# s-will/BiAlign

Measured on AMD Instinct MI355X. Metric: giga-DP-cells/sec, higher is better.
Workload: dtype int32

## Files before the change

bialign_amd/csrc/bialign_host.hpp:

```cpp
#pragma once
#include "bialign_plan.hpp"

#include <algorithm>
#include <cstdarg>
#include <cstdio>
#include <cstdlib>
#include <cstring>
#include <memory>
#include <mutex>
#include <numeric>
#include <string>
#include <type_traits>
#include <vector>

namespace bialign {

#define HIP_TRY(expr)                                                                 \
  do {                                                                                \
    hipError_t e_ = (expr);                                                           \
    if (e_ != hipSuccess)                                                             \
      return fail(BIALIGN_E_DEVICE, "%s failed: %s (%s:%d)", #expr, hipGetErrorString(e_), \
                  __FILE__, __LINE__);                                                \
  } while (0)

template <typename T>
struct DevBuf {
  T* p = nullptr;
  size_t n = 0;
  ~DevBuf() { release(); }
  void release() {
    if (p) (void)hipFree(p);
    p = nullptr;
    n = 0;
  }
  void swap(DevBuf& o) {
    std::swap(p, o.p);
    std::swap(n, o.n);
  }
  hipError_t alloc(size_t count) {
    release();
    n = count;
    return hipMalloc(reinterpret_cast<void**>(&p), std::max<size_t>(count, 1) * sizeof(T));
  }
  hipError_t upload(const T* src, size_t count, hipStream_t s) {
    hipError_t e = alloc(count);
    if (e != hipSuccess || count == 0) return e;
    return hipMemcpyAsync(p, src, count * sizeof(T), hipMemcpyHostToDevice, s);
  }
};

}

using bialign::DevBuf;
using bialign::DeviceBatch;
using bialign::PairDesc;
using bialign::TraceState;

struct bialign_engine {
  int device = 0;
  int num_cu = 256;
  hipStream_t stream = nullptr;
  hipStream_t copy_stream = nullptr;
  hipEvent_t ev[4] = {nullptr, nullptr, nullptr, nullptr};
  int live_batches = 0;
  bool closing = false;
  DevBuf<int32_t> layer_cache;
  DevBuf<int32_t> layer_cache2;
  DevBuf<int32_t> tab_cache;
};

struct bialign_batch : bialign::BatchPlan {
  bialign_engine* eng = nullptr;
  DevBuf<PairDesc> d_pairs;
  DevBuf<int32_t> d_order, d_s1, d_s2, d_layers, d_scores, d_tlen, d_complete, d_err, d_prog;
  DevBuf<int32_t> d_span;
  DevBuf<unsigned long long> d_end_key;
  int last_team = 1;
  int xcu_resident[4] = {-1, -1, -1, -1};
  bool used_xcu = false;
  bool no_xcu = false;
  int recovered = 0;
  int xcu_spin_limit = 1 << 20;
  uint32_t pending_flags = 0;
  bool used_pack = false;
  bool packed_layers = false;
  DevBuf<uint8_t> d_seq_a, d_cls_a, d_seq_b, d_cls_b, d_trace;
  DevBuf<int32_t> d_tab;
  DevBuf<double> d_feat_a, d_feat_b;
  int64_t feat_tot_a = 0, feat_tot_b = 0;
  DevBuf<int32_t> d_mu1;
  DevBuf<int64_t> d_mu1_off;
  std::vector<hipEvent_t> build_evs;
  double build_ms = 0;
  int build_launches = 0;
  DevBuf<uint8_t> d_null_seq, d_null_cls;
  DevBuf<int64_t> d_null_off;
  DevBuf<double> d_null_feat;
  DevBuf<int32_t> d_null_tab;
  DevBuf<int64_t> d_null_tab_off;
  DevBuf<uint16_t> d_null_perm;
  DevBuf<int32_t> d_null_obs;
  DevBuf<bialign_null_stats> d_null_stats;
  hipEvent_t null_evs[4] = {nullptr, nullptr, nullptr, nullptr};
  double shuffle_ms = 0, stats_ms = 0;
  int32_t null_model = BIALIGN_NULL_MONO;
  DevBuf<TraceState> d_tstate;
  bool hits_on = false;
  bialign_hit_spec hit_spec{};
  DevBuf<int32_t> d_hit_profile, d_hit_head, d_hit_rec, d_hit_walks;
  DevBuf<int64_t> d_hit_prof_off;
  DevBuf<uint8_t> d_hit_trace;
  std::vector<int64_t> hit_prof_off;
  int hit_mask_words = 0;
  int64_t hit_bytes = 0;
  std::vector<hipEvent_t> hit_evs;
  bool hits_pending = false;
  bool hits_ran = false;
  double search_ms = 0;
  void release_hits() {
    hits_on = hits_ran = false;
    for (DevBuf<int32_t>* d : {&d_hit_profile, &d_hit_head, &d_hit_rec, &d_hit_walks}) d->release();
    d_hit_prof_off.release();
    d_hit_trace.release();
    hit_bytes = 0;
  }
  bialign_timing timing{};
  bool ran = false, ran_trace = false;
  bool pending = false, pending_trace = false;
  std::vector<hipEvent_t> evs;
  hipEvent_t uploaded = nullptr;
  ~bialign_batch() {
    for (hipEvent_t e : evs)
      if (e) (void)hipEventDestroy(e);
    for (hipEvent_t e : build_evs)
      if (e) (void)hipEventDestroy(e);
    for (hipEvent_t e : null_evs)
      if (e) (void)hipEventDestroy(e);
    for (hipEvent_t e : hit_evs)
      if (e) (void)hipEventDestroy(e);
    if (uploaded) (void)hipEventDestroy(uploaded);
  }

  DeviceBatch view() const {
    DeviceBatch v{};
    v.pairs = d_pairs.p;
    v.order = d_order.p;
    v.seq_a = d_seq_a.p; v.cls_a = d_cls_a.p; v.seq_b = d_seq_b.p; v.cls_b = d_cls_b.p;
    v.s1 = d_s1.p; v.s2 = d_s2.p;
    v.k1 = k1; v.k2 = k2;
    v.beta = prm.gap_opening_cost; v.gamma = prm.gap_cost; v.delta = prm.shift_cost;
    v.layers = d_layers.p;
    v.scores = d_scores.p;
    v.trace = d_trace.p;
    v.trace_len = d_tlen.p;
    v.complete = d_complete.p;
    v.errflag = d_err.p;
    v.dense_tab = (dense || dense1) ? d_tab.p : nullptr;
    v.dense_forms = (dense ? 1 : 0) | (dense1 ? 2 : 0);
    v.scratch = d_layers.p;
    v.wide_ring = ring_dwords.empty() ? nullptr : d_layers.p + max_chunk_dwords;
    v.wide_score_only = !ring_dwords.empty() && lean ? 1 : 0;
    v.tstate = d_tstate.p;
    v.resw_k = level_trace ? wide_seg : resw_k;
    v.wide_s = S;
    v.prio_mode = getenv("BIALIGN_PRIO") ? atoi(getenv("BIALIGN_PRIO")) : 1;
    v.spin_limit = 1 << 20;
    v.free_ends = mode == bialign::AlignMode::Fit       ? bialign::FREE_B_ENDS
                  : mode == bialign::AlignMode::Overlap ? bialign::FREE_B_ENDS | bialign::FREE_A_ENDS
                                                        : 0;
    v.local = mode == bialign::AlignMode::Local;
    v.reserved0 = nullptr;
    v.span = d_span.p;
    v.end_key = d_end_key.p;
    return v;
  }
};

namespace bialign {

int xcu_serial_begin(bialign_engine* e);
int xcu_serial_end(bialign_engine* e);

int launch_build_mu2(bialign_batch* b, int first, int count);

int launch_shuffle_null(bialign_batch* b, int first, int count);
int launch_permute_tables(bialign_batch* b, int first, int count);
int launch_null_stats(bialign_batch* b, const int32_t* d_observed);

template <typename... P>
hipError_t allow_lds(void (*kern)(P...), size_t lds) {
  if (lds <= 64 * 1024) return hipSuccess;
  return hipFuncSetAttribute(reinterpret_cast<const void*>(kern), hipFuncAttributeMaxDynamicSharedMemorySize, (int)lds);
}
template <typename... P, typename... A>
hipError_t try_launch(void (*kern)(P...), dim3 grid, dim3 block, size_t lds, hipStream_t st, const A&... args) {
  if (hipError_t e = allow_lds(kern, lds)) return e;
  hipLaunchKernelGGL(kern, grid, block, lds, st, args...);
  return hipGetLastError();
}
template <typename... P, typename... A>
int launch(void (*kern)(P...), dim3 grid, dim3 block, size_t lds, hipStream_t st, const A&... args) {
  HIP_TRY(try_launch(kern, grid, block, lds, st, args...));
  return BIALIGN_OK;
}

template <typename... P, typename... X>
int launch_team(bialign_batch* b, void (*kern)(P...), dim3 grid, dim3 block, size_t lds, DeviceBatch w, int count,
                bool serial, const X&... extra) {
  const size_t words = (size_t)count * PROG_WORDS;
  if (b->d_prog.n < words) HIP_TRY(b->d_prog.alloc(words));
  HIP_TRY(hipMemsetAsync(b->d_prog.p, 0, words * sizeof(int32_t), b->eng->stream));
  w.prog = b->d_prog.p;
  w.spin_limit = b->xcu_spin_limit;
  if (!serial) return launch(kern, grid, block, lds, b->eng->stream, w, extra...);
  b->used_xcu = true;
  if (int rc = xcu_serial_begin(b->eng)) return rc;
  const hipError_t launched = try_launch(kern, grid, block, lds, b->eng->stream, w, extra...);
  const int rc = xcu_serial_end(b->eng);
  if (launched == hipSuccess && rc) return rc;
  HIP_TRY(launched);
  return BIALIGN_OK;
}

template <typename... P>
int xcu_resident(const bialign_batch* b, void (*kern)(P...), int block, size_t lds) {
  int per_cu = 0;
  if (allow_lds(kern, lds) != hipSuccess ||
      hipOccupancyMaxActiveBlocksPerMultiprocessor(&per_cu, reinterpret_cast<const void*>(kern), block, lds) != hipSuccess) {
    (void)hipGetLastError();
    return 0;
  }
  return per_cu * b->eng->num_cu;
}
template <typename... P>
int xcu_resident_cached(bialign_batch* b, int slot, void (*kern)(P...), int block, size_t lds) {
  if (b->no_xcu) return 0;
  int& cached = b->xcu_resident[slot];
  if (cached < 0) cached = xcu_resident(b, kern, block, lds);
  return cached;
}

template <unsigned MASK, unsigned F = 0, typename Fn>
int with_flags(unsigned flags, Fn&& fn) {
  if constexpr (MASK == 0) {
    return fn(std::integral_constant<unsigned, F>{});
  } else {
    constexpr unsigned BIT = MASK & (~MASK + 1);
    return (flags & BIT) ? with_flags<(MASK & ~BIT), (F | BIT)>(flags, fn) : with_flags<(MASK & ~BIT), F>(flags, fn);
  }
}

enum FillFlags : unsigned {
  F_XCU = 1,
  F_DENSE = 2,
  F_LEAN = 4,
  F_RESW = 8,
  F_PACK = 16,
  F_DENSE1 = 32,
  F_BETA_ANY = 64,
  F_LOCAL = 128,
};
enum TraceFlags : unsigned {
  T_TRACE = 1,
  T_STRIP = 2,
  T_WIDE = 4,
  T_PACK = 8,
  T_DENSE1 = 16,
  T_LEVEL = 32,
};

constexpr bool fill_affine_exists(int S, int TW, unsigned F) {
  const bool xcu = F & F_XCU, dense = F & (F_DENSE | F_DENSE1), pack = F & F_PACK;
  if (F & F_LOCAL) return !(F & (F_XCU | F_PACK | F_RESW | F_BETA_ANY)) && (TW == 1 || (TW == 4 && S <= 3));
  if (pack && (S < 1 || S > BIALIGN_MAX_SHIFT_PACKED || (F & (F_LEAN | F_DENSE1)))) return false;
  if (F & (F_RESW | F_BETA_ANY)) return TW == 1 && !xcu && !pack && !((F & F_RESW) && (F & F_LEAN));
  if (TW == 1) return !xcu || !dense || S <= 3;
  if (TW == 8) return !dense && (xcu ? S == 2 : S <= 2);
  return (TW == 4 || TW == 2) && !xcu && S <= 3;
}
constexpr bool fill_linear_exists(int TW, unsigned F) {
  if (F & (F_PACK | F_BETA_ANY)) return false;
  if (F & F_LOCAL) return !(F & (F_XCU | F_RESW)) && (TW == 1 || (TW == 4 && !(F & (F_DENSE | F_DENSE1))));
  if (F & (F_RESW | F_XCU)) return TW == 1 && (F & (F_RESW | F_XCU)) != (F_RESW | F_XCU) && !((F & F_RESW) && (F & F_LEAN));
  return TW == 1 || TW == 2 || (!(F & (F_DENSE | F_DENSE1)) && (TW == 4 || TW == 8));
}
constexpr bool fill_slim_exists(int S, unsigned F) { return S == 1 && (F == F_LEAN || F == F_PACK); }
constexpr bool traceback_exists(bool affine, int S, unsigned F) {
  if ((F & T_PACK) && (!affine || S < 1 || S > BIALIGN_MAX_SHIFT_PACKED || (F & ~(T_PACK | T_TRACE)))) return false;
  if (F & T_LEVEL) return S == 0 && (F & ~T_DENSE1) == (T_LEVEL | T_TRACE);
  if (F & T_STRIP) return (F & T_TRACE) && !(F & T_WIDE);
  return !(F & T_DENSE1) || (F & T_TRACE);
}

template <int S, int TW, unsigned F>
auto fill_affine_of() {
  static_assert(fill_affine_exists(S, TW, F), "not in the instantiation plan");
  return fill_affine_kernel<S, !(F & F_BETA_ANY), TW, (F & F_XCU) != 0, (F & F_DENSE) != 0, (F & F_LEAN) != 0, (F & F_RESW) != 0,
                            (F & F_PACK) != 0, (F & F_DENSE1) != 0, (F & F_LOCAL) != 0>;
}
template <int S, int TW, unsigned F>
auto fill_linear_of() {
  static_assert(fill_linear_exists(TW, F), "not in the instantiation plan");
  return fill_linear_kernel<S, TW, (F & F_DENSE) != 0, (F & F_LEAN) != 0, (F & F_RESW) != 0, (F & F_XCU) != 0, (F & F_DENSE1) != 0,
                            (F & F_LOCAL) != 0>;
}
template <int S, unsigned F>
auto traceback_affine_of() {
  static_assert(traceback_exists(true, S, F), "not in the instantiation plan");
  return traceback_affine_kernel<S, (F & T_TRACE) != 0, (F & T_STRIP) != 0, (F & T_WIDE) != 0, (F & T_PACK) != 0, (F & T_DENSE1) != 0,
                                 (F & T_LEVEL) != 0>;
}
template <int S, unsigned F>
auto traceback_linear_of() {
  static_assert(traceback_exists(false, S, F), "not in the instantiation plan");
  return traceback_linear_kernel<S, (F & T_TRACE) != 0, (F & T_STRIP) != 0, (F & T_WIDE) != 0, (F & T_DENSE1) != 0, (F & T_LEVEL) != 0>;
}

inline unsigned fill_flags(const bialign_batch* b) {
  return (b->dense ? F_DENSE : 0u) | (b->dense1 ? F_DENSE1 : 0u) | (b->lean ? F_LEAN : 0u) | (b->pack_now() ? F_PACK : 0u) |
         (b->affine && b->prm.gap_opening_cost > 0 ? F_BETA_ANY : 0u);
}
template <int S, int TW>
size_t fill_lds(const bialign_batch* b, bool affine) {
  return (affine && S == 2 && TW == 8) ? b->lds_diet8 : b->lds_base + (size_t)TW * b->lds_per_wave;
}

template <int S, int TW, unsigned F>
int launch_fill_affine_t(bialign_batch* b, const DeviceBatch& v, int first, int count, int gw) {
  constexpr bool XCU = (F & F_XCU) != 0, PACK = (F & F_PACK) != 0;
  DeviceBatch w = v;
  w.order = v.order + first;
  w.team = gw;
  b->packed_layers = PACK;
  if (PACK) b->used_pack = true;
  b->last_team = XCU ? -TW * gw : TW;
  const dim3 grid(count * (XCU ? gw : 1)), block(64 * TW);
  if (XCU) return launch_team(b, fill_affine_of<S, TW, F>(), grid, block, fill_lds<S, TW>(b, true), w, count, true);
  return launch(fill_affine_of<S, TW, F>(), grid, block, fill_lds<S, TW>(b, true), b->eng->stream, w);
}

template <int S, int TW, bool LEAN>
int launch_fill_affine_slim_t(bialign_batch* b, const DeviceBatch& v, int first, int count) {
  constexpr int PPW = 12 / TW;
  DeviceBatch w = v;
  w.order = v.order + first;
  w.team = 1;
  w.launch_pairs = count;
  w.slim_code_bytes = (int32_t)b->lds_slim_codes;
  b->packed_layers = !LEAN;
  if (!LEAN) b->used_pack = true;
  b->last_team = TW;
  return launch(fill_affine_slim_kernel<S, TW, PPW, LEAN>, dim3((count + PPW - 1) / PPW), dim3(64 * 12), b->lds_slim(TW),
                b->eng->stream, w);
}

template <int S, bool LEAN>
int launch_fill_affine_slim(bialign_batch* b, const DeviceBatch& v, int first, int count, int tw) {
  switch (tw) {
    case 2: return launch_fill_affine_slim_t<S, 2, LEAN>(b, v, first, count);
    case 3: return launch_fill_affine_slim_t<S, 3, LEAN>(b, v, first, count);
    case 6: return launch_fill_affine_slim_t<S, 6, LEAN>(b, v, first, count);
    case 12: return launch_fill_affine_slim_t<S, 12, LEAN>(b, v, first, count);
  }
  return fail(BIALIGN_E_UNSUPPORTED, "no three-waves-per-SIMD sweep for max_shift %d, team %d", S, tw);
}

template <int S, int TW, unsigned F>
int xcu_resident_affine(bialign_batch* b) {
  constexpr unsigned Q = (F & ~F_PACK) | F_XCU;
  if constexpr (fill_affine_exists(S, TW, Q)) {
    if (TW == 8 && !diet8_available(*b)) return 0;
    return xcu_resident_cached(b, ((F & F_LEAN) ? 1 : 0) + (TW == 8 ? 2 : 0), fill_affine_of<S, TW, Q>(), 64 * TW, fill_lds<S, TW>(b, true));
  } else {
    return 0;
  }
}

template <int S, int TW, unsigned F>
bool fill_affine_rung(bialign_batch* b, const DeviceBatch& v, int first, int count, const TeamShape& ts, int* rc) {
  if constexpr (fill_affine_exists(S, TW, F)) {
    constexpr bool XCU = (F & F_XCU) != 0;
    if (XCU ? !(ts.gw > 1 && (TW == 1 || ts.tw == TW)) : ts.tw < TW) return false;
    *rc = launch_fill_affine_t<S, TW, F>(b, v, first, count, XCU ? ts.gw : 1);
    return true;
  } else {
    return false;
  }
}

template <int S>
int launch_fill_affine(bialign_batch* b, const DeviceBatch& v, int first, int count) {
  return with_flags<F_DENSE | F_LEAN | F_PACK | F_DENSE1 | F_BETA_ANY>(fill_flags(b), [&](auto flags) -> int {
    constexpr unsigned F = decltype(flags)::value;
    if constexpr (!fill_affine_exists(S, 1, F)) {
      return fail(BIALIGN_E_UNSUPPORTED, "no affine sweep for max_shift %d in form %u", S, F);
    } else {
      TeamShape ts;
      if constexpr (!(F & F_BETA_ANY)) ts = team_shape(*b, first, count, b->eng->num_cu, xcu_resident_affine<S, 1, F>(b), xcu_resident_affine<S, 8, F>(b));
      if constexpr (fill_slim_exists(S, F)) {
        if (ts.slim) return launch_fill_affine_slim<S, (F & F_LEAN) != 0>(b, v, first, count, ts.tw);
      }
      int rc = BIALIGN_OK;
      (void)(fill_affine_rung<S, 8, F | F_XCU>(b, v, first, count, ts, &rc) || fill_affine_rung<S, 1, F | F_XCU>(b, v, first, count, ts, &rc) ||
             fill_affine_rung<S, 8, F>(b, v, first, count, ts, &rc) || fill_affine_rung<S, 4, F>(b, v, first, count, ts, &rc) ||
             fill_affine_rung<S, 2, F>(b, v, first, count, ts, &rc) || fill_affine_rung<S, 1, F>(b, v, first, count, ts, &rc));
      return rc;
    }
  });
}

template <int S>
int launch_fill_affine_local(bialign_batch* b, const DeviceBatch& v, int first, int count) {
  return with_flags<F_DENSE | F_LEAN | F_DENSE1>(fill_flags(b) & ~(unsigned)(F_PACK | F_BETA_ANY), [&](auto flags) -> int {
    constexpr unsigned F = decltype(flags)::value | F_LOCAL;
    const TeamShape ts = team_shape(*b, first, count, b->eng->num_cu, 0);
    int rc = BIALIGN_OK;
    (void)(fill_affine_rung<S, 4, F>(b, v, first, count, ts, &rc) || fill_affine_rung<S, 1, F>(b, v, first, count, ts, &rc));
    return rc;
  });
}

template <int S>
int launch_resweep_affine(bialign_batch* b, const DeviceBatch& v, int first, int count) {
  DeviceBatch w = v;
  w.order = v.order + first;
  w.team = 1;
  return with_flags<F_DENSE | F_DENSE1 | F_BETA_ANY>(fill_flags(b), [&](auto flags) -> int {
    return launch(fill_affine_of<S, 1, decltype(flags)::value | F_RESW>(), dim3(count * b->resw_k), dim3(64), fill_lds<S, 1>(b, true),
                  b->eng->stream, w);
  });
}

inline unsigned trace_flags(const bialign_batch* b, bool do_trace) {
  return (do_trace ? T_TRACE : 0u) | (b->dense1 && do_trace ? T_DENSE1 : 0u) | (b->packed_layers ? T_PACK : 0u);
}
template <typename... P>
int launch_traceback_kernel(const bialign_batch* b, void (*kern)(P...), bool do_trace, const DeviceBatch& v, int first, int count) {
  DeviceBatch w = v;
  w.order = v.order + first;
  return launch(kern, dim3(count), dim3(64), do_trace ? b->lds_trace : 0, b->eng->stream, w, count);
}

constexpr bool traceback_fast_exists(int S, unsigned F) { return F == (T_TRACE | T_PACK) && traceback_exists(true, S, F); }
template <int S>
bool trace_fast_admits(const PairDesc& d) {
  using TF = TraceFast<S>;
  return Pack<S>::pair_dwords(d.G, d.P, d.m) < (int64_t(1) << 31) &&
         (2 * (int64_t)d.P + Geo<S>::MAXOFF + TF::W + 2) * TF::RECB < (int64_t(1) << 32);
}
constexpr int TRACE_FAST_TBUF_MAX = 16 * 1024;
template <int S>
size_t trace_fast_lds(const bialign_batch* b, int first, int count, int* tbuf) {
  const char* sw = getenv("BIALIGN_TRACE_FAST");
  if ((sw && atoi(sw) == 0) || b->dense || b->dense1 || b->wide || b->lean) return 0;
  if (b->free_ends()) return 0;
  int cap = 0;
  for (int t = first; t < first + count; ++t) {
    const PairDesc& d = b->pairs[b->order[t]];
    if (!trace_fast_admits<S>(d)) return 0;
    cap = std::max(cap, d.trace_cap);
  }
  int want = std::min((cap + 63) & ~63, TRACE_FAST_TBUF_MAX);
  if (const char* e = getenv("BIALIGN_TRACE_LDS")) want = std::min(want, std::max(64, atoi(e) & ~63));
  const size_t fixed = ((b->lds_trace + 15) & ~size_t(15)) + TraceFast<S>::TAB_BYTES;
  if (fixed + 64 > 160 * 1024) return 0;
  *tbuf = (int)std::min<size_t>(want, (160 * 1024 - fixed) & ~size_t(63));
  return fixed + *tbuf;
}

template <int S>
int launch_traceback_affine(const bialign_batch* b, const DeviceBatch& v, int first, int count, bool do_trace) {
  return with_flags<T_TRACE | T_PACK | T_DENSE1>(trace_flags(b, do_trace), [&](auto flags) -> int {
    constexpr unsigned F = decltype(flags)::value;
    if constexpr (traceback_fast_exists(S, F)) {
      int tbuf = 0;
      if (const size_t lds = trace_fast_lds<S>(b, first, count, &tbuf)) {
        DeviceBatch w = v;
        w.order = v.order + first;
        return launch(traceback_affine_fast_kernel<S>, dim3(count), dim3(64), lds, b->eng->stream, w, count, tbuf);
      }
    }
    if constexpr (traceback_exists(true, S, F)) return launch_traceback_kernel(b, traceback_affine_of<S, F>(), do_trace, v, first, count);
    else return fail(BIALIGN_E_UNSUPPORTED, "no affine traceback for max_shift %d in form %u", S, F);
  });
}
template <int S>
int launch_traceback_affine_strip(const bialign_batch* b, const DeviceBatch& v, int first, int count) {
  return b->dense1 ? launch_traceback_kernel(b, traceback_affine_of<S, T_TRACE | T_STRIP | T_DENSE1>(), true, v, first, count)
                   : launch_traceback_kernel(b, traceback_affine_of<S, T_TRACE | T_STRIP>(), true, v, first, count);
}

template <int S, int TW, unsigned F>
int launch_fill_linear_t(bialign_batch* b, const DeviceBatch& v, int first, int count, int gw) {
  constexpr bool XCU = (F & F_XCU) != 0;
  DeviceBatch w = v;
  w.order = v.order + first;
  w.team = gw;
  b->packed_layers = false;
  b->last_team = XCU ? -gw : TW;
  const dim3 grid(count * (XCU ? gw : 1)), block(64 * TW);
  if (XCU) return launch_team(b, fill_linear_of<S, TW, F>(), grid, block, fill_lds<S, TW>(b, false), w, count, true);
  return launch(fill_linear_of<S, TW, F>(), grid, block, fill_lds<S, TW>(b, false), b->eng->stream, w);
}

template <int S, int TW, unsigned F>
bool fill_linear_rung(bialign_batch* b, const DeviceBatch& v, int first, int count, const TeamShape& ts, int* rc) {
  if constexpr (fill_linear_exists(TW, F)) {
    constexpr bool XCU = (F & F_XCU) != 0;
    if (XCU ? ts.gw <= 1 : ts.tw < TW) return false;
    *rc = launch_fill_linear_t<S, TW, F>(b, v, first, count, XCU ? ts.gw : 1);
    return true;
  } else {
    return false;
  }
}

template <int S>
int launch_fill_linear(bialign_batch* b, const DeviceBatch& v, int first, int count) {
  return with_flags<F_DENSE | F_LEAN | F_DENSE1>(fill_flags(b), [&](auto flags) -> int {
    constexpr unsigned F = decltype(flags)::value;
    const int resident = xcu_resident_cached(b, (F & F_LEAN) ? 1 : 0, fill_linear_of<S, 1, F | F_XCU>(), 64, fill_lds<S, 1>(b, false));
    const TeamShape ts = team_shape(*b, first, count, b->eng->num_cu, resident);
    int rc = BIALIGN_OK;
    (void)(fill_linear_rung<S, 1, F | F_XCU>(b, v, first, count, ts, &rc) || fill_linear_rung<S, 8, F>(b, v, first, count, ts, &rc) ||
           fill_linear_rung<S, 4, F>(b, v, first, count, ts, &rc) || fill_linear_rung<S, 2, F>(b, v, first, count, ts, &rc) ||
           fill_linear_rung<S, 1, F>(b, v, first, count, ts, &rc));
    return rc;
  });
}

template <int S>
int launch_fill_linear_local(bialign_batch* b, const DeviceBatch& v, int first, int count) {
  return with_flags<F_DENSE | F_LEAN | F_DENSE1>(fill_flags(b), [&](auto flags) -> int {
    constexpr unsigned F = decltype(flags)::value | F_LOCAL;
    const TeamShape ts = team_shape(*b, first, count, b->eng->num_cu, 0);
    int rc = BIALIGN_OK;
    (void)(fill_linear_rung<S, 4, F>(b, v, first, count, ts, &rc) || fill_linear_rung<S, 1, F>(b, v, first, count, ts, &rc));
    return rc;
  });
}

template <int S>
int launch_resweep_linear(bialign_batch* b, const DeviceBatch& v, int first, int count) {
  DeviceBatch w = v;
  w.order = v.order + first;
  return with_flags<F_DENSE | F_DENSE1>(fill_flags(b), [&](auto flags) -> int {
    return launch(fill_linear_of<S, 1, decltype(flags)::value | F_RESW>(), dim3(count * b->resw_k), dim3(64), fill_lds<S, 1>(b, false),
                  b->eng->stream, w);
  });
}

template <int S>
int launch_traceback_linear(const bialign_batch* b, const DeviceBatch& v, int first, int count, bool do_trace) {
  return with_flags<T_TRACE | T_DENSE1>(trace_flags(b, do_trace), [&](auto flags) -> int {
    constexpr unsigned F = decltype(flags)::value;
    if constexpr (traceback_exists(false, S, F)) return launch_traceback_kernel(b, traceback_linear_of<S, F>(), do_trace, v, first, count);
    else return fail(BIALIGN_E_UNSUPPORTED, "no one-layer traceback for max_shift %d in form %u", S, F);
  });
}
template <int S>
int launch_traceback_linear_strip(const bialign_batch* b, const DeviceBatch& v, int first, int count) {
  return b->dense1 ? launch_traceback_kernel(b, traceback_linear_of<S, T_TRACE | T_STRIP | T_DENSE1>(), true, v, first, count)
                   : launch_traceback_kernel(b, traceback_linear_of<S, T_TRACE | T_STRIP>(), true, v, first, count);
}

template <int S, int NL>
int launch_dump(const bialign_batch* b, const DeviceBatch& v, int pid, int32_t* d_out) {
  if constexpr (S >= 1 && S <= BIALIGN_MAX_SHIFT_PACKED && NL == 9) {
    if (b->packed_layers) return launch(dump_layers_kernel<S, NL, true>, dim3(256), dim3(256), 0, b->eng->stream, v, pid, d_out);
  }
  return launch(dump_layers_kernel<S, NL>, dim3(256), dim3(256), 0, b->eng->stream, v, pid, d_out);
}

int launch_fill_wide(bialign_batch* b, const DeviceBatch& v, int first, int count);
int launch_traceback_wide(const bialign_batch* b, const DeviceBatch& v, int first, int count, bool do_trace);
int launch_segment_wide(bialign_batch* b, const DeviceBatch& v, int first, int count);
int launch_traceback_level(const bialign_batch* b, const DeviceBatch& v, int first, int count);
int launch_dump_wide(const bialign_batch* b, const DeviceBatch& v, int pid, int32_t* d_out);

#define BIALIGN_INST_KIND0(S, X)                                                                \
  X template int launch_fill_affine<S>(bialign_batch*, const DeviceBatch&, int, int);          \
  X template int launch_resweep_affine<S>(bialign_batch*, const DeviceBatch&, int, int);
#define BIALIGN_INST_KIND1(S, X)                                                                         \
  X template int launch_fill_linear<S>(bialign_batch*, const DeviceBatch&, int, int);                   \
  X template int launch_traceback_affine<S>(const bialign_batch*, const DeviceBatch&, int, int, bool);  \
  X template int launch_traceback_affine_strip<S>(const bialign_batch*, const DeviceBatch&, int, int);  \
  X template int launch_traceback_linear<S>(const bialign_batch*, const DeviceBatch&, int, int, bool);  \
  X template int launch_resweep_linear<S>(bialign_batch*, const DeviceBatch&, int, int);                \
  X template int launch_traceback_linear_strip<S>(const bialign_batch*, const DeviceBatch&, int, int);  \
  X template int launch_dump<S, 9>(const bialign_batch*, const DeviceBatch&, int, int32_t*);            \
  X template int launch_dump<S, 1>(const bialign_batch*, const DeviceBatch&, int, int32_t*);

#define BIALIGN_INST_KIND2(S, X)                                                                \
  X template int launch_fill_affine_local<S>(bialign_batch*, const DeviceBatch&, int, int);    \
  X template int launch_fill_linear_local<S>(bialign_batch*, const DeviceBatch&, int, int);

#ifndef BIALIGN_TU_S
BIALIGN_FOR_EACH_S(BIALIGN_INST_KIND0, extern)
BIALIGN_FOR_EACH_S(BIALIGN_INST_KIND1, extern)
BIALIGN_FOR_EACH_S(BIALIGN_INST_KIND2, extern)
#endif

}
```

bialign_amd/csrc/bialign_trace_fast.hpp:

```cpp
#pragma once

namespace bialign {

template <int S>
struct TraceFast {
  using PK = Pack<S>;
  static constexpr int W = 2 * S + 1, RR = Geo<S>::RR;
  static constexpr int RECB = PK::RECDW * 4;
  static constexpr int ENTRIES = 9 * W * 16;
  static constexpr int TAIL_SHIFT = PK::TAILDW == 2 ? 1 : 2;
  static constexpr uint32_t NONE = 15;
  struct Entry {
    uint32_t lo;
    int32_t cst, da, db;
  };
  static constexpr int TAB_BYTES = ENTRIES * (int)sizeof(Entry);
  static constexpr uint32_t NEED_I = 1u << 20, NEED_J = 1u << 21, NEED_K = 1u << 22, NEED_L = 1u << 23;
  static constexpr uint32_t NEED_ALO = 1u << 24, NEED_AHI = 1u << 25;
  static constexpr uint32_t NEVER = 1u << 26;
  __host__ __device__ static constexpr int shift_hd(int hU, int hV) { return hU == hV ? 0 : ((hU == 2 || hV == 2) ? 1 : 2); }
  __host__ __device__ static inline Entry entry(int st, int b0, int c, int beta, int gamma, int delta) {
    if (c >= 15) return Entry{NEVER | NONE << 4, 0, 0, 0};
    const int hU = st / 3, hV = st - 3 * hU;
    const int u0 = hU >= 1, u1 = hU != 1, v0 = hV >= 1, v1 = hV != 1;
    const int grp = c < 9 ? 1 : (c < 12 ? 2 : 3);
    const int hfree = grp == 2 ? 2 - (c - 9) : 2 - (c - 12);
    const int o0 = grp == 2 ? 0 : u0, o1 = grp == 2 ? 0 : u1;
    const int o2 = grp == 3 ? 0 : v0, o3 = grp == 3 ? 0 : v1;
    const int ss = grp == 1 ? c : (grp == 2 ? 3 * hU + hfree : 3 * hfree + hV);
    const int ra = ss / 3, rb = ss - 3 * ra;
    const int openU = (hU != 2 && ra != hU) ? beta : 0, openV = (hV != 2 && rb != hV) ? beta : 0;
    const int gU = hU == 2 ? 0 : gamma, gV = hV == 2 ? 0 : gamma;
    const int cst = grp == 1   ? delta * shift_hd(hU, hV) + gU + gV + openU + openV
                    : grp == 2 ? delta * (v0 + v1) + gV + openV
                               : delta * (u0 + u1) + gU + openU;
    const uint32_t m1 = grp != 2 && hU == 2, m2 = grp != 3 && hV == 2;
    const int r0 = ra >= 1, r1 = ra != 1, r2 = rb >= 1, r3 = rb != 1;
    const int inc0 = (o0 - o2) + (r0 - r2), inc1 = (o1 - o3) + (r1 - r3);
    const uint32_t code = (uint32_t)(o0 * 8 + o1 * 4 + o2 * 2 + o3);
    const int b = b0 + o1 - o3;
    if (b < 0 || b >= W) return Entry{NEVER | NONE << 4 | code, cst, 0, 0};
    const int v = b * 9 + ss, h = PK::hw(v), d = h >> 1;
    const bool anchor = v == PK::ANCHOR, tail = !anchor && d >= 4 * PK::NCH;
    const uint32_t half = anchor ? 2u : (uint32_t)(h & 1);
    const int hpos = anchor ? 0 : (tail ? PK::NCH * Rec<S, 9>::CH + (d - 4 * PK::NCH) : (d >> 2) * Rec<S, 9>::CH + (d & 3));
    const int da = o0 - o2;
    const uint32_t need = (o0 ? NEED_I : 0) | (o1 ? NEED_J : 0) | (o2 ? NEED_K : 0) | (o3 ? NEED_L : 0) | (da < 0 ? NEED_ALO : 0) |
                          (da > 0 ? NEED_AHI : 0);
    const uint32_t lo = code | (uint32_t)ss << 4 | m1 << 8 | m2 << 9 | ((uint32_t)inc0 & 7u) << 10 | ((uint32_t)inc1 & 7u) << 13 |
                        (tail ? 1u : 0u) << 16 | half << 17 | (pack_corner(W, ss, b) ? 1u : 0u) << 19 | need;
    const int drec = (da - o1 - 2 * o0) * RECB, dslot16 = (da - o0 * W) * 16;
    return Entry{lo, cst, drec + dslot16, tail ? drec + hpos * 4 + dslot16 / (1 << TAIL_SHIFT) : drec + dslot16 + hpos * 4};
  }
  __host__ __device__ static inline uint32_t deny(int i, int j, int k, int l) {
    const int a0 = k - i + S;
    return NEVER | (i > 0 ? 0 : NEED_I) | (j > 0 ? 0 : NEED_J) | (k > 0 ? 0 : NEED_K) | (l > 0 ? 0 : NEED_L) | (a0 > 0 ? 0 : NEED_ALO) |
           (a0 < W - 1 ? 0 : NEED_AHI);
  }
  struct Pos {
    int strip, il;
    int64_t row;
    __host__ __device__ static inline Pos at(int i, int P) {
      Pos p;
      p.strip = i / RR;
      p.il = i - p.strip * RR + 1;
      p.row = ((int64_t)p.strip - 1) * P * RECB;
      return p;
    }
    __host__ __device__ inline void step_up(int P) {
      if (--il == 0) {
        il = RR;
        --strip;
        row -= (int64_t)P * RECB;
      }
    }
  };
  struct Col {
    bool fast;
    uint32_t u16, u8;
  };
  __host__ __device__ static inline Col column(int strip, int il, int j, int a0, int P, int m) {
    const bool up = il == 1;
    const int tl = j + 2 * il;
    Col c;
    c.fast = strip - (up ? 1 : 0) >= PK::Q0 && tl >= PK::LO + 3 && tl <= m - S - W + 1 - (up ? 2 * RR - 2 : 0);
    const uint32_t rec = (uint32_t)P * RECB + (uint32_t)(tl + a0) * RECB, slot16 = (uint32_t)(il * W + a0) * 16;
    c.u16 = rec + slot16 - W * 16;
    c.u8 = rec + (slot16 >> TAIL_SHIFT) - ((W * 16) >> TAIL_SHIFT);
    return c;
  }
  __host__ __device__ static inline uint32_t up16(int P) { return (uint32_t)(2 * RR * RECB + RR * W * 16) - (uint32_t)P * RECB; }
  __host__ __device__ static inline uint32_t up8(int P) { return (uint32_t)(2 * RR * RECB + ((RR * W * 16) >> TAIL_SHIFT)) - (uint32_t)P * RECB; }
  struct Off {
    uint32_t base, word;
  };
  __host__ __device__ static inline Off offsets(const Entry& e, const Col& c, bool up, int P) {
    const bool tail = (e.lo >> 16) & 1;
    Off o{c.u16 + (uint32_t)e.da, (tail ? c.u8 : c.u16) + (uint32_t)e.db};
    if (up && (e.lo & 8)) {
      o.base += up16(P);
      o.word += tail ? up8(P) : up16(P);
    }
    return o;
  }
};

template <int S>
__global__ void __launch_bounds__(64) traceback_affine_fast_kernel(const DeviceBatch A, int npairs, int tbuf_bytes) {
  using TF = TraceFast<S>;
  typedef typename TF::Entry Entry;
  const int pid = A.order[blockIdx.x];
  const PairDesc pd = A.pairs[pid];
  const int n = pd.n, m = pd.m, P = pd.P, cap = pd.trace_cap;
  const int c = threadIdx.x;
  constexpr int BIG = 0x7fffffff;
  constexpr int W = TF::W, RR = TF::RR;
  extern __shared__ __align__(16) int32_t smem[];
  const int32_t* const pbase = A.layers + pd.layer_off;

  const int endv = c < 9 ? packed_cell<S>(A.layers, pd, n, m, S, S, c) : -BIG;
  const int best = __builtin_amdgcn_readfirstlane(-wave_min16(-endv));
  if (c == 0) A.scores[pid] = best;
  const int skey = (c < 9 && endv == best) ? (shift_of(c / 3, c % 3) << 4 | c) : BIG;
  int st = __builtin_amdgcn_readfirstlane(wave_min16(skey)) & 15;
  int cur = best;

  const TraceInputs in = stage_trace_inputs<false>(A, pd, smem);
  const int staged = ((A.k1 * A.k1 + A.k2 * A.k2) * 4 + 2 * (code_pad(n) + code_pad(m)) + 15) & ~15;
  Entry* const tab = reinterpret_cast<Entry*>(reinterpret_cast<char*>(smem) + staged);
  uint8_t* const tbuf = reinterpret_cast<uint8_t*>(tab + TF::ENTRIES);
  for (int e = c; e < TF::ENTRIES; e += 64) tab[e] = TF::entry(e / (16 * W), (e >> 4) % W, e & 15, A.beta, A.gamma, A.delta);
  __syncthreads();

  uint8_t* const out = A.trace + pd.trace_off;
  int i = n, j = m, k = n, l = m, d0 = 0, d1 = 0, len = 0, complete = 0, flushed = 0;
  typename TF::Pos pos = TF::Pos::at(n, P);
  const char* rowp = reinterpret_cast<const char*>(pbase) + pos.row;
  const uint32_t prb = (uint32_t)P * TF::RECB, up16 = TF::up16(P), up8 = TF::up8(P);
  const Entry* const tabc = tab + (c < 15 ? c : 15);
  const int k1 = A.k1, k2 = A.k2;
  int vz = 0;
  asm volatile("" : "+v"(vz));
  int room = min(tbuf_bytes, cap);
  auto flush = [&](int cnt) {
    __syncthreads();
    for (int y = c; y < cnt; y += 64) out[cap - 1 - flushed - y] = tbuf[y];
    __syncthreads();
    flushed += cnt;
  };
  while (true) {
    if ((i | j | k | l | (st ^ 8)) == 0) { complete = 1; break; }
    const Entry E = tabc[(st * W + (l - j + S)) * 16];
    int ca = in.sa[i - 1 + vz], cb = in.sb[j - 1 + vz], cc = in.ca[k - 1 + vz], cd = in.cb[l - 1 + vz];
    const uint32_t lo = E.lo;
    const int a0 = k - i + S;
    uint32_t deny = TF::NEVER | (a0 > 0 ? 0 : TF::NEED_ALO) | (a0 < W - 1 ? 0 : TF::NEED_AHI);
    const bool edge = min(min(i, j), min(k, l)) == 0;
    if (edge) deny = TF::deny(i, j, k, l);
    const bool ok = (lo & deny) == 0;
    const typename TF::Col col = TF::column(pos.strip, pos.il, j, a0, P, m);
    int ld = 0;
    if (col.fast) {
      if (ok) {
        const bool tail = (lo >> 16) & 1;
        uint32_t ob = col.u16 + (uint32_t)E.da, ow = (tail ? col.u8 : col.u16) + (uint32_t)E.db;
        if (pos.il == 1 && (lo & 8)) {
          ob += up16;
          ow += tail ? up8 : up16;
        }
        const int base = *reinterpret_cast<const int32_t*>(rowp + ob);
        const uint32_t word = *reinterpret_cast<const uint32_t*>(rowp + ow);
        const uint32_t half = (lo >> 17) & 3;
        const uint32_t e = Pack<S>::offset_of(half == 1 ? word >> 16 : word & 0xffffu, base);
        ld = base + (int)e;
        if (((lo >> 19) & 1) && e == 0xffffu) ld = NEG;
        if (half == 2) ld = base + 0x8000;
      }
    } else if (ok) {
      const int o0 = (lo >> 3) & 1, o1 = (lo >> 2) & 1, o2 = (lo >> 1) & 1, o3 = lo & 1;
      ld = packed_load<S>(pbase, packed_addr<S>(pd, i - o0, j - o1, a0 + o0 - o2, (l - j + S) + o1 - o3, (lo >> 4) & 15));
    }
    bool z1 = false, z2 = false;
    if (edge) {
      z1 = i < 1 || j < 1;
      z2 = k < 1 || l < 1;
      if (z1) ca = cb = 0;
      if (z2) cc = cd = 0;
    }
    int mu1 = in.s1[__umul24(ca, k1) + cb], mu2 = in.s2[__umul24(cc, k2) + cd];
    if (z1) mu1 = 0;
    if (z2) mu2 = 0;
    const int sc = E.cst + (((lo >> 8) & 1) ? mu1 : 0) + (((lo >> 9) & 1) ? mu2 : 0);
    const int t0 = d0 + ((int)(lo << 19) >> 29), t1 = d1 + ((int)(lo << 16) >> 29);
    const int key = (ok && ld + sc == cur) ? ((abs(t0) + abs(t1)) << 16 | abs(t1) << 8 | c) : BIG;
    const int kmin = __builtin_amdgcn_readfirstlane(wave_min16(key));
    if (kmin == BIG) break;
    const int pick = kmin & 63;
    const int cs = __builtin_amdgcn_readlane((int)lo, pick);
    cur = __builtin_amdgcn_readlane(ld, pick);
    st = (cs >> 4) & 15;
    const int q0 = (cs >> 3) & 1, q1 = (cs >> 2) & 1, q2 = (cs >> 1) & 1, q3 = cs & 1;
    d0 += q0 - q2;
    d1 += q1 - q3;
    if (room > 0) {
      if (c == 0) tbuf[len - flushed] = (uint8_t)(cs & 15);
      if (--room == 0) {
        if (len + 1 - flushed == tbuf_bytes) flush(tbuf_bytes);
        room = min(tbuf_bytes, cap - (len + 1));
      }
    }
    ++len;
    i -= q0; j -= q1; k -= q2; l -= q3;
    if (q0) {
      const int strip_was = pos.strip;
      pos.step_up(P);
      if (pos.strip != strip_was) rowp -= prb;
    }
  }
  if (len > cap) len = cap;
  if (flushed == 0) {
    __syncthreads();
    for (int x = c; x < len; x += 64) out[x] = tbuf[len - 1 - x];
  } else {
    flush(len - flushed);
    const int sh = cap - len;
    if (sh > 0) {
      __builtin_amdgcn_s_waitcnt(0);
      __syncthreads();
      for (int x0 = 0; x0 < len; x0 += 64) {
        const int x = x0 + c;
        const uint8_t t = x < len ? out[sh + x] : 0;
        if (x < len) out[x] = t;
      }
    }
  }
  if (c == 0) {
    A.trace_len[pid] = len;
    A.complete[pid] = complete;
  }
}

}
```

Before: 210.5.

## Prefetch traceback window records into an LDS ring via async global-to-LDS loads

Adds a TraceWindow ring buffer in LDS for the fast affine traceback. Upcoming packed DP records along the traceback path are prefetched ahead of use with global_load_lds_dwordx4, so the serial traceback loop reads from LDS instead of waiting on dependent global loads. This trades extra LDS per block and a per-step issue/wait cost for hiding global memory latency. A host heuristic enables it only when the added LDS does not cut the needed occupancy.

```diff
diff --git a/bialign_amd/csrc/bialign_host.hpp b/bialign_amd/csrc/bialign_host.hpp
--- a/bialign_amd/csrc/bialign_host.hpp
+++ b/bialign_amd/csrc/bialign_host.hpp
@@ -450,7 +450,21 @@
 }
 constexpr int TRACE_FAST_TBUF_MAX = 16 * 1024;
 template <int S>
-size_t trace_fast_lds(const bialign_batch* b, int first, int count, int* tbuf) {
+int trace_window_records(const bialign_batch* b, int count, size_t fixed, int tbuf) {
+  using TW = TraceWindow<S>;
+  const char* sw = getenv("BIALIGN_TRACE_WINDOW");
+  if (sw && atoi(sw) == 0) return 0;
+  int k = TW::K;
+  if (const char* e = getenv("BIALIGN_TRACE_WINDOW_K"))
+    while (k > TW::KMIN && k > atoi(e)) k /= 2;
+  const size_t lds = 160 * 1024, with = fixed + TW::lds_bytes(k);
+  if (with > 64 * 1024 || with + 64 > lds) return 0;
+  const size_t res_with = lds / (with + tbuf), res_without = lds / (fixed + tbuf);
+  const size_t needed = ((size_t)count + b->eng->num_cu - 1) / std::max(b->eng->num_cu, 1);
+  return res_with >= std::min(res_without, needed) ? k : 0;
+}
+template <int S>
+size_t trace_fast_lds(const bialign_batch* b, int first, int count, int* tbuf, int* wk) {
   const char* sw = getenv("BIALIGN_TRACE_FAST");
   if ((sw && atoi(sw) == 0) || b->dense || b->dense1 || b->wide || b->lean) return 0;
   if (b->free_ends()) return 0;
@@ -462,8 +476,11 @@
   }
   int want = std::min((cap + 63) & ~63, TRACE_FAST_TBUF_MAX);
   if (const char* e = getenv("BIALIGN_TRACE_LDS")) want = std::min(want, std::max(64, atoi(e) & ~63));
-  const size_t fixed = ((b->lds_trace + 15) & ~size_t(15)) + TraceFast<S>::TAB_BYTES;
+  size_t fixed = ((b->lds_trace + 15) & ~size_t(15)) + TraceFast<S>::TAB_BYTES;
   if (fixed + 64 > 160 * 1024) return 0;
+  *wk = 0;
+  if constexpr (TraceWindow<S>::EXISTS) *wk = trace_window_records<S>(b, count, fixed, want);
+  if (*wk) fixed += TraceWindow<S>::lds_bytes(*wk);
   *tbuf = (int)std::min<size_t>(want, (160 * 1024 - fixed) & ~size_t(63));
   return fixed + *tbuf;
 }
@@ -473,11 +490,13 @@
   return with_flags<T_TRACE | T_PACK | T_DENSE1>(trace_flags(b, do_trace), [&](auto flags) -> int {
     constexpr unsigned F = decltype(flags)::value;
     if constexpr (traceback_fast_exists(S, F)) {
-      int tbuf = 0;
-      if (const size_t lds = trace_fast_lds<S>(b, first, count, &tbuf)) {
+      int tbuf = 0, wk = 0;
+      if (const size_t lds = trace_fast_lds<S>(b, first, count, &tbuf, &wk)) {
         DeviceBatch w = v;
         w.order = v.order + first;
-        return launch(traceback_affine_fast_kernel<S>, dim3(count), dim3(64), lds, b->eng->stream, w, count, tbuf);
+        if constexpr (TraceWindow<S>::EXISTS)
+          if (wk) return launch(traceback_affine_fast_kernel<S, true>, dim3(count), dim3(64), lds, b->eng->stream, w, count, tbuf, wk);
+        return launch(traceback_affine_fast_kernel<S, false>, dim3(count), dim3(64), lds, b->eng->stream, w, count, tbuf, 0);
       }
     }
     if constexpr (traceback_exists(true, S, F)) return launch_traceback_kernel(b, traceback_affine_of<S, F>(), do_trace, v, first, count);
diff --git a/bialign_amd/csrc/bialign_trace_fast.hpp b/bialign_amd/csrc/bialign_trace_fast.hpp
--- a/bialign_amd/csrc/bialign_trace_fast.hpp
+++ b/bialign_amd/csrc/bialign_trace_fast.hpp
@@ -106,8 +106,80 @@
 };
 
 template <int S>
-__global__ void __launch_bounds__(64) traceback_affine_fast_kernel(const DeviceBatch A, int npairs, int tbuf_bytes) {
+struct TraceWindow {
   using TF = TraceFast<S>;
+  using PK = Pack<S>;
+  using R_ = Rec<S, 9>;
+  static constexpr int W = TF::W, RECB = TF::RECB;
+  static constexpr int RECS_PER_COL = 3;
+  static constexpr int SPAN = RECS_PER_COL + 1;
+  static constexpr int WS = S == 1 ? 16 : 32;
+  __host__ __device__ static constexpr int drift(int x) { return (W * x + 1) / 2 + (W - 1) * (W - 2) / 2; }
+  __host__ __device__ static constexpr int lead_max() {
+    int d = -1;
+    while (drift(d + 1 + RECS_PER_COL) + W + 2 <= WS) ++d;
+    return d;
+  }
+  static constexpr int D = lead_max() < 4 ? lead_max() : 4;
+  static constexpr bool EXISTS = D >= 0 && (PK::TAILDW == 0 || PK::TAILDW == 2);
+  static constexpr int K = 8, KMIN = SPAN;
+  static_assert(!EXISTS || (K >= D + SPAN && (K & (K - 1)) == 0 && (KMIN & (KMIN - 1)) == 0), "ring too short for the lead");
+  static_assert(!EXISTS || WS <= R_::SLP, "a window record is wider than a record");
+  static constexpr int NPIECE16 = PK::NCH * WS + WS * PK::TAILDW / 4;
+  static constexpr int NDMA = (NPIECE16 + 63) / 64;
+  static constexpr int RB = NDMA * 1024;
+  static constexpr int TAIL_AT = PK::NCH * WS * 16;
+  static constexpr int WTAB_BYTES = TF::ENTRIES * 4;
+  __host__ __device__ static constexpr int lds_bytes(int k) { return WTAB_BYTES + k * RB; }
+  __host__ __device__ static constexpr int lead(int k) { return k - SPAN < D ? k - SPAN : D; }
+  __host__ __device__ static inline int slot_lo(int s) {
+    const int lo = (s + 2 - WS) & ~1;
+    return lo > 0 ? lo : 0;
+  }
+  struct LaneSrc {
+    uint32_t base, u, sh;
+  };
+  __host__ __device__ static inline LaneSrc lane_src(int d, int lane) {
+    const int q = d * 64 + lane < NPIECE16 ? d * 64 + lane : NPIECE16 - 1;
+    const int p = q / WS, u = q - p * WS;
+    if (p < PK::NCH) return LaneSrc{(uint32_t)(p * R_::CH * 4), (uint32_t)u, 4u};
+    return LaneSrc{(uint32_t)(PK::NCH * R_::CH * 4), (uint32_t)(2 * u), 3u};
+  }
+  __host__ __device__ static inline uint32_t src_off(const LaneSrc& c, int slo) {
+    return c.base + (((uint32_t)slo + ((c.u - (uint32_t)slo) & (WS - 1))) << c.sh);
+  }
+  __host__ __device__ static inline uint32_t ring_byte(int r, int k) { return (uint32_t)(r & (k - 1)) * RB; }
+  __host__ __device__ static inline uint32_t wentry(int st, int b0, int c) {
+    if (c >= 15) return 0;
+    const typename TF::Entry e = TF::entry(st, b0, c, 0, 0, 0);
+    if (((e.lo >> 4) & 15) == TF::NONE) return 0;
+    const int o0 = (e.lo >> 3) & 1, o1 = (e.lo >> 2) & 1, o2 = (e.lo >> 1) & 1, o3 = e.lo & 1;
+    const int v = (b0 + o1 - o3) * 9 + (int)((e.lo >> 4) & 15);
+    uint32_t woff = 0;
+    if (v != PK::ANCHOR) {
+      const int d = PK::hw(v) >> 1;
+      woff = d >= 4 * PK::NCH ? TAIL_AT + (d - 4 * PK::NCH) * 4 : (d >> 2) * WS * 16 + (d & 3) * 4;
+    }
+    return woff | (uint32_t)(o0 + o1 + o2) << 16 | (uint32_t)((W - 1) * o0 + o2) << 20;
+  }
+  __host__ __device__ static inline typename TF::Off addr(uint32_t we, bool tail, int T, int s, int k) {
+    const uint32_t ring = ring_byte(T - (int)((we >> 16) & 3), k), u = (uint32_t)(s - (int)((we >> 20) & 15)) & (WS - 1);
+    return typename TF::Off{ring + u * 16, ring + (we & 0xfffu) + (tail ? u * 8 : u * 16)};
+  }
+  __host__ __device__ static inline bool full_lead(int T, int next) { return T - RECS_PER_COL - next == D; }
+  __host__ __device__ static inline int may_pend(int T, int next) { return full_lead(T, next) ? D * NDMA : 0; }
+};
+
+template <int N>
+__device__ __forceinline__ void trace_window_wait() {
+  asm volatile("s_waitcnt vmcnt(%0)" ::"n"(N) : "memory");
+}
+
+template <int S, bool WIN = false>
+__global__ void __launch_bounds__(64) traceback_affine_fast_kernel(const DeviceBatch A, int npairs, int tbuf_bytes, int wk) {
+  using TF = TraceFast<S>;
+  using TW = TraceWindow<S>;
+  static_assert(!WIN || TW::EXISTS, "no window at this max_shift");
   typedef typename TF::Entry Entry;
   const int pid = A.order[blockIdx.x];
   const PairDesc pd = A.pairs[pid];
@@ -128,8 +200,12 @@
   const TraceInputs in = stage_trace_inputs<false>(A, pd, smem);
   const int staged = ((A.k1 * A.k1 + A.k2 * A.k2) * 4 + 2 * (code_pad(n) + code_pad(m)) + 15) & ~15;
   Entry* const tab = reinterpret_cast<Entry*>(reinterpret_cast<char*>(smem) + staged);
-  uint8_t* const tbuf = reinterpret_cast<uint8_t*>(tab + TF::ENTRIES);
+  uint32_t* const wtab = reinterpret_cast<uint32_t*>(tab + TF::ENTRIES);
+  const char* const wring = reinterpret_cast<const char*>(wtab + TF::ENTRIES);
+  uint8_t* const tbuf = WIN ? reinterpret_cast<uint8_t*>(const_cast<char*>(wring) + wk * TW::RB) : reinterpret_cast<uint8_t*>(tab + TF::ENTRIES);
   for (int e = c; e < TF::ENTRIES; e += 64) tab[e] = TF::entry(e / (16 * W), (e >> 4) % W, e & 15, A.beta, A.gamma, A.delta);
+  if constexpr (WIN)
+    for (int e = c; e < TF::ENTRIES; e += 64) wtab[e] = TW::wentry(e / (16 * W), (e >> 4) % W, e & 15);
   __syncthreads();
 
   uint8_t* const out = A.trace + pd.trace_off;
@@ -148,9 +224,39 @@
     __syncthreads();
     flushed += cnt;
   };
+#if defined(BIALIGN_EXP) && BIALIGN_EXP == 10
+  int whits = 0;
+#endif
+  [[maybe_unused]] int wnext = 0;
+  [[maybe_unused]] bool wlive = false;
+  [[maybe_unused]] const int wlead = TW::lead(wk);
+  [[maybe_unused]] const uint32_t wlds = (uint32_t)(uintptr_t)(__attribute__((address_space(3))) int32_t*)smem + (uint32_t)(wring - reinterpret_cast<const char*>(smem));
+  [[maybe_unused]] typename TW::LaneSrc wsrc[TW::NDMA];
+  if constexpr (WIN) {
+#pragma unroll
+    for (int d = 0; d < TW::NDMA; ++d) wsrc[d] = TW::lane_src(d, c);
+  }
+  [[maybe_unused]] auto wissue = [&](int r, int s) {
+    const char* const base = rowp + prb + (uint32_t)r * (uint32_t)TF::RECB;
+    const uint32_t dst0 = wlds + TW::ring_byte(r, wk);
+    const int slo = TW::slot_lo(s);
+#pragma unroll
+    for (int d = 0; d < TW::NDMA; ++d) {
+      const uint32_t off = TW::src_off(wsrc[d], slo), dst = dst0 + d * 1024;
+      uint32_t keep;
+      asm volatile(
+          "s_mov_b32 %0, m0\n\ts_mov_b32 m0, %2\n\ts_nop 0\n\t"
+          "global_load_lds_dwordx4 %1, %3\n\ts_mov_b32 m0, %0"
+          : "=&s"(keep)
+          : "v"(off), "s"(dst), "s"(base)
+          : "memory");
+    }
+  };
   while (true) {
     if ((i | j | k | l | (st ^ 8)) == 0) { complete = 1; break; }
     const Entry E = tabc[(st * W + (l - j + S)) * 16];
+    [[maybe_unused]] uint32_t we = 0;
+    if constexpr (WIN) we = (wtab + (c < 15 ? c : 15))[(st * W + (l - j + S)) * 16];
     int ca = in.sa[i - 1 + vz], cb = in.sb[j - 1 + vz], cc = in.ca[k - 1 + vz], cd = in.cb[l - 1 + vz];
     const uint32_t lo = E.lo;
     const int a0 = k - i + S;
@@ -160,7 +266,30 @@
     const bool ok = (lo & deny) == 0;
     const typename TF::Col col = TF::column(pos.strip, pos.il, j, a0, P, m);
     int ld = 0;
-    if (col.fast) {
+    auto value = [&](int base, uint32_t word) {
+      const uint32_t half = (lo >> 17) & 3;
+      const uint32_t e = Pack<S>::offset_of(half == 1 ? word >> 16 : word & 0xffffu, base);
+      int v = base + (int)e;
+      if (((lo >> 19) & 1) && e == 0xffffu) v = NEG;
+      if (half == 2) v = base + 0x8000;
+      return v;
+    };
+    [[maybe_unused]] bool hit = false;
+    [[maybe_unused]] const int wT = j + 2 * pos.il + a0;
+    if constexpr (WIN) hit = col.fast && wlive && pos.il >= 2 && wT - TW::RECS_PER_COL >= wnext;
+    if (WIN && hit) {
+      if constexpr (WIN) {
+#if defined(BIALIGN_EXP) && BIALIGN_EXP == 10
+        ++whits;
+#endif
+        if (TW::full_lead(wT, wnext)) trace_window_wait<TW::D * TW::NDMA>();
+        else trace_window_wait<0>();
+        if (ok) {
+          const typename TF::Off o = TW::addr(we, (lo >> 16) & 1, wT, (pos.il - 1) * W + a0, wk);
+          ld = value(*reinterpret_cast<const int32_t*>(wring + o.base), *reinterpret_cast<const uint32_t*>(wring + o.word));
+        }
+      }
+    } else if (col.fast) {
       if (ok) {
         const bool tail = (lo >> 16) & 1;
         uint32_t ob = col.u16 + (uint32_t)E.da, ow = (tail ? col.u8 : col.u16) + (uint32_t)E.db;
@@ -168,17 +297,12 @@
           ob += up16;
           ow += tail ? up8 : up16;
         }
-        const int base = *reinterpret_cast<const int32_t*>(rowp + ob);
-        const uint32_t word = *reinterpret_cast<const uint32_t*>(rowp + ow);
-        const uint32_t half = (lo >> 17) & 3;
-        const uint32_t e = Pack<S>::offset_of(half == 1 ? word >> 16 : word & 0xffffu, base);
-        ld = base + (int)e;
-        if (((lo >> 19) & 1) && e == 0xffffu) ld = NEG;
-        if (half == 2) ld = base + 0x8000;
+        ld = value(*reinterpret_cast<const int32_t*>(rowp + ob), *reinterpret_cast<const uint32_t*>(rowp + ow));
       }
     } else if (ok) {
       const int o0 = (lo >> 3) & 1, o1 = (lo >> 2) & 1, o2 = (lo >> 1) & 1, o3 = lo & 1;
       ld = packed_load<S>(pbase, packed_addr<S>(pd, i - o0, j - o1, a0 + o0 - o2, (l - j + S) + o1 - o3, (lo >> 4) & 15));
+      if constexpr (WIN) asm volatile("" ::"v"(ld));
     }
     bool z1 = false, z2 = false;
     if (edge) {
@@ -214,9 +338,25 @@
     if (q0) {
       const int strip_was = pos.strip;
       pos.step_up(P);
-      if (pos.strip != strip_was) rowp -= prb;
-    }
-  }
+      if (pos.strip != strip_was) {
+        rowp -= prb;
+        if constexpr (WIN) wlive = false;
+      }
+    }
+    if constexpr (WIN) {
+      const int a1 = k - i + S, Tn = j + 2 * pos.il + a1;
+      if (!wlive && pos.il >= 2) {
+        wlive = true;
+        wnext = Tn + 1;
+      }
+      if (wlive) {
+        const int low = max(Tn - TW::RECS_PER_COL - wlead, 0);
+        for (int r = wnext - 1; r >= low; --r) wissue(r, (pos.il - 1) * W + a1);
+        wnext = min(wnext, low);
+      }
+    }
+  }
+  if constexpr (WIN) trace_window_wait<0>();
   if (len > cap) len = cap;
   if (flushed == 0) {
     __syncthreads();
@@ -237,6 +377,9 @@
   if (c == 0) {
     A.trace_len[pid] = len;
     A.complete[pid] = complete;
+#if defined(BIALIGN_EXP) && BIALIGN_EXP == 10
+    if constexpr (WIN) A.scores[pid] = whits;
+#endif
   }
 }
 
```

Result: faster. 213.3 (median of 6 runs) (+1.3%).
